# rampasek/GraphGPS

Measured on NVIDIA H100. Metric: graphs/sec GPSLayer fwd+bwd, higher is better.
Workload: dtype f32

## Files before the change

graphgps_b200/_lib.py:

```python
from __future__ import annotations

import ctypes as C
import os

import torch

_HERE = os.path.dirname(os.path.abspath(__file__))
LIB_PATH = os.path.join(_HERE, "libgps_b200.so")

GPS_OK, GPS_ERR_ARG, GPS_ERR_UNSUPPORTED, GPS_ERR_CUDA = 0, -1, -2, -3
LOCAL = {"None": 0, "CustomGatedGCN": 1, "GINE": 2, "GCN": 3, "GAT": 4, "GENConv": 5, "PNA": 6}
GLOBAL = {"None": 0, "Transformer": 1, "Performer": 2, "BigBird": 3}
GLOBAL_BIGBIRD = GLOBAL["BigBird"]
BIGBIRD_ACT = {"relu": 0, "sigmoid": 1}
ACT = {"relu": 0, "gelu": 1}
PRECISION = {"fp32": 0, "bf16": 1}
NORM = {"batch": 0, "none": 1}
FLAG_GRADS_ZEROED, FLAG_GRADS_ACCUMULATE = 1, 2

_fp = C.c_void_p


class GpsGraph(C.Structure):
    _fields_ = [("N", C.c_int64), ("E", C.c_int64), ("B", C.c_int64),
# ... 247 lines not shown
    "gps_pna_aggregate_forward": (C.c_int, [C.POINTER(GpsGraph), _i64, _fp, _fp, _i64, _fp, _fp, _fp, _fp]),
    "gps_pna_aggregate_backward": (C.c_int, [C.POINTER(GpsGraph), _i64, _fp, _fp, _fp, _fp, _fp, _i64, _fp, _fp]),
    "gps_performer_prep": (C.c_int, [C.POINTER(GpsGraph), _i64, _i64, _i64, _fp, _fp, _fp, _fp, _fp, _fp]),
    "gps_performer_features_forward": (C.c_int, [C.POINTER(GpsGraph), _i64, _i64, _i64, _fp, _fp, _fp, _fp, _fp, _fp,
                                                 _fp, _fp]),
    "gps_performer_attention_forward": (C.c_int, [C.POINTER(GpsGraph), _i64, _i64, _i64, _i32, _fp, _fp, _fp, _fp, _fp,
                                                  _fp, _fp, _fp]),
    "gps_performer_attention_backward": (C.c_int, [C.POINTER(GpsGraph), _i64, _i64, _i64, _i32, _fp, _fp, _fp, _fp,
                                                   _fp, _fp, _fp, _fp, _fp, _fp, _fp, _fp, _fp, _fp, _fp]),
    "gps_performer_features_backward": (C.c_int, [C.POINTER(GpsGraph), _i64, _i64, _i64, _i32, _fp, _fp, _fp, _fp, _fp,
                                                  _fp, _fp, _fp, _fp, _fp, _fp, _fp, _fp]),
    "gps_attention_forward": (C.c_int, [C.POINTER(GpsGraph), _i64, _i64, _fp, _fp, _fp, _i64, _fp, _i64, _fp,
                                        _f32, _u64, _u64, _fp]),
    "gps_attention_backward": (C.c_int, [C.POINTER(GpsGraph), _i64, _i64, _fp, _fp, _fp, _i64, _fp, _fp, _i64,
                                         _fp, _fp, _fp, _fp, _fp, _i64, _f32, _u64, _u64, _fp]),
    "gps_attention_forward_tc": (C.c_int, [C.POINTER(GpsGraph), _i64, _i64, _fp, _fp, _i64, _fp, _i64, _fp, _f32, _u64, _u64,
                                           _i32, _fp]),
    "gps_attention_forward_biased": (C.c_int, [C.POINTER(GpsGraph), _i64, _i64, _fp, _fp, _fp, _i64, _fp, _i64, _fp,
                                               _f32, _u64, _u64, C.POINTER(GpsAttnBias), _fp]),
    "gps_attention_forward_tc_biased": (C.c_int, [C.POINTER(GpsGraph), _i64, _i64, _fp, _fp, _i64, _fp, _i64, _fp, _f32,
                                                  _u64, _u64, _i32, C.POINTER(GpsAttnBias), _fp]),
    "gps_attention_backward_biased": (C.c_int, [C.POINTER(GpsGraph), _i64, _i64, _fp, _fp, _fp, _i64, _fp, _fp, _i64,
                                                _fp, _fp, _fp, _fp, _fp, _i64, _f32, _u64, _u64, C.POINTER(GpsAttnBias),
                                                _fp]),
    "gps_dropout_mask": (C.c_int, [_fp, _i64, _i64, _f32, _u64, _u64, _i32, _fp]),
    "gps_to_planes": (C.c_int, [_fp, _i64, _i64, _i64, _fp, _fp, _i64, _fp]),
    "gps_gemm_planes": (C.c_int, [_fp, _fp, _i64, _i32, _fp, _fp, _i64, _i32, _fp, _i64, _fp, _fp, _i64, _i64, _i64, _i64,
                                  _i32, _i32, _fp, _fp]),
    "gps_gemm_epilogue": (C.c_int, [C.POINTER(GpsGemmArgs), _i32, _fp]),
    "gps_fallback_count": (C.c_ulonglong, []),
    "gps_launch_count": (C.c_ulonglong, []),
    "gps_debug_set": (None, [C.c_int]),
    "gps_debug_tma": (None, [C.c_int, _fp]),
    "gps_debug_attn": (None, [_fp]),
}

_lib = None


def load():
    global _lib
    if _lib is not None:
        return _lib
    if not os.path.exists(LIB_PATH):
        raise RuntimeError(
            f"{LIB_PATH} not found: build it with `python -m graphgps_b200.build` "
            "(nvcc, sm_90a). graphgps_b200 has no CPU/eager fallback.")
    lib = C.CDLL(LIB_PATH)
    for name, (res, args) in SYMBOLS.items():
        fn = getattr(lib, name)
        fn.restype = res
        fn.argtypes = args
    if lib.gps_abi_version() != 4:
        raise RuntimeError("libgps_b200.so ABI version mismatch")
    _lib = lib
    return lib


class GpsError(RuntimeError):
    pass


def check(rc: int, what: str):
    if rc == GPS_OK:
        return
    msg = load().gps_last_error().decode("utf-8", "replace")
# ... 10 lines not shown
```

graphgps_b200/csrc/gemm.cuh:

```cuda
#pragma once
#include <cuda.h>

#include "common.cuh"

namespace gps {

struct GemmParams {
  int M = 0, N = 0, K = 0;
  const float* A = nullptr; int lda = 0; int ta = 0;
  const float* B = nullptr; int ldb = 0; int tb = 0;
  float* C = nullptr; int ldc = 0;
  const float* bias = nullptr;
  float* C_pre = nullptr; int ldpre = 0;
  int act = -1;
  const float* mask_src = nullptr; int ldmask = 0; int mask_act = -1;
  int mask_is_post = 0;
  float p_drop = 0.f; uint64_t seed = 0, offset = 0; int site = 0;
  const unsigned long long* offset_dev = nullptr;
  float p_drop2 = 0.f; int site2 = 0;
  const float* R1 = nullptr; int ldr1 = 0;
  const float* R2 = nullptr; int ldr2 = 0;
  double* stats = nullptr;
  int splitk = 1;
  float* colsum_a = nullptr;
  int precision = GPS_PREC_FP32;
  Planes Ap, Bp, Cp;
  int cp_hd = 0, cp_hd_pad = 0;
};

struct ToPlanesItem { const float* src; int64_t ld; int rows; int cols; Planes dst; };
int to_planes(const ToPlanesItem* items, int n, cudaStream_t stream);
int gemm_tma(const GemmParams& p, cudaStream_t stream);
int make_tensor_map(const __nv_bfloat16* hi, const __nv_bfloat16* lo, int planes, int64_t rows, int64_t cols, int64_t ld,
                    int box_rows, CUtensorMap* out);
void gemm_tma_set_force_bn(int bn);
void gemm_tma_set_trace(unsigned long long* buf);

int gemm_simt(const GemmParams& p, cudaStream_t stream);
int gemm_tc(const GemmParams& p, cudaStream_t stream);
void gemm_tc_set_debug(int v);
int gemm(const GemmParams& p, cudaStream_t stream);

}
```

graphgps_b200/csrc/gemm_tma.cu:

```cuda
#include <cooperative_groups.h>
#include <cuda.h>
#include <cuda_bf16.h>

#include <mutex>
#include <unordered_map>

#include "gemm.cuh"
#include "tc_ptx.cuh"

namespace gps {

namespace {

using namespace tc;
namespace cgrp = cooperative_groups;

constexpr int BM = 128;
constexpr int BK = 64;
constexpr int kEpiWarps = 8;
constexpr int kTmaWarp = 8;
constexpr int kThreads = 288;
constexpr int kATile = BM * BK * 2;
constexpr int kBlock = 64 * BK * 2;
constexpr int kMaxSplits = 8;

struct TmaArgs {
  GemmParams p;
  int BN, nb_blocks, stages, kb_per_split, planes;
  unsigned long long* trace;
};

__device__ __forceinline__ unsigned long long gtimer() {
  unsigned long long t;
  asm volatile("mov.u64 %0, %globaltimer;" : "=l"(t));
  return t;
}
#define GPS_TRACE(slot)                                                                         \
  do {                                                                                          \
    if (a.trace && cta_lin < 256) a.trace[cta_lin * 16 + (slot)] = gtimer();                    \
  } while (0)

template <bool A_MN, bool B_MN, int BN_T, bool SPLIT>
__global__ void __launch_bounds__(kThreads, BN_T == 64 ? 2 : 1)
k_gemm_tma(const __grid_constant__ CUtensorMap tmA, const __grid_constant__ CUtensorMap tmB, const TmaArgs a) {
  extern __shared__ __align__(1024) uint8_t smem_raw[];
  const GemmParams& p = a.p;
  uint8_t* smem = reinterpret_cast<uint8_t*>((reinterpret_cast<uintptr_t>(smem_raw) + 1023) & ~(uintptr_t)1023);
  const int planes = a.planes;
  const int b_tile = B_MN ? a.nb_blocks * kBlock : BN_T * 128;
  const int stage_bytes = planes * (kATile + b_tile);
  const int S = a.stages;
  uint64_t* bars = reinterpret_cast<uint64_t*>(smem + (size_t)S * stage_bytes);
  float* red = reinterpret_cast<float*>(bars + 2 * S + 2);
  float* ctot = red + 16 * 16 * 8;
  const int nsplit = (int)gridDim.z;

  const int tid = threadIdx.x, warp = tid >> 5, lane = tid & 31;
  const int m0 = blockIdx.y * BM, n0 = blockIdx.x * a.BN;
  const int nkb_total = (p.K + BK - 1) / BK;
  const int kb_begin = blockIdx.z * a.kb_per_split;
  const int kb_end = min(nkb_total, kb_begin + a.kb_per_split);
  const int nkb = kb_end - kb_begin;
  const bool do_colsum = A_MN && p.colsum_a != nullptr && blockIdx.x == 0;
  const int cta_lin = (blockIdx.z * gridDim.y + blockIdx.y) * gridDim.x + blockIdx.x;

  if (tid == 0) {
    GPS_TRACE(0);
    if (a.trace && cta_lin < 256) {
      unsigned smid;
// ... 108 lines not shown
      __syncwarp();
      if (i > 0 && lane == 0) mbar_arrive(smem_u32(&bars[S + (i - 1) % S]));
    }
    wgmma_wait<0>();
    reg_fence<BN_T / 2>(acc);
    if (tid == 0) GPS_TRACE(4);
    if (do_colsum) {
#pragma unroll
      for (int e = 0; e < 8; ++e) red[(kq * 16 + cm) * 8 + e] = csum[e];
    }
    asm volatile("bar.sync 1, 256;" ::: "memory");
    if (do_colsum && tid < 128) {
      const int cmr = tid >> 3, e = tid & 7;
      float tot = 0.f;
#pragma unroll
      for (int o = 0; o < 16; ++o) tot += red[(o * 16 + cmr) * 8 + e];
      const int gm = m0 + cmr * 8 + e;
      if (nsplit > 1) ctot[cmr * 8 + e] = tot;
      else if (gm < p.M) atomicAdd(&p.colsum_a[gm], tot);
    }
    if (tid == 0) GPS_TRACE(5);
    float* stage = reinterpret_cast<float*>(smem);
    const int sld = a.BN + 4;
    {
      const int r = wg * 64 + (warp & 3) * 16 + (lane >> 2);
      const int c = 2 * (lane & 3);
#pragma unroll
      for (int j = 0; j < BN_T / 8; ++j) {
        *reinterpret_cast<float2*>(stage + r * sld + 8 * j + c) = make_float2(acc[4 * j], acc[4 * j + 1]);
        *reinterpret_cast<float2*>(stage + (r + 8) * sld + 8 * j + c) = make_float2(acc[4 * j + 2], acc[4 * j + 3]);
      }
    }
    asm volatile("bar.sync 1, 256;" ::: "memory");
    const int RB = (BM + nsplit - 1) / nsplit;
    const int lo = (int)blockIdx.z * RB, hi = min(BM, lo + RB);
    if (nsplit > 1) {
      cgrp::cluster_group cluster = cgrp::this_cluster();
      cluster.sync();
      const int c4n = a.BN >> 2;
      for (int idx = tid; idx < (hi - lo) * c4n; idx += kEpiWarps * 32) {
        const int r = lo + idx / c4n, c = (idx % c4n) * 4;
        float4 sum = f4zero();
        for (int k = 0; k < nsplit; ++k)
          sum = f4add(sum, *reinterpret_cast<const float4*>(cluster.map_shared_rank(stage, k) + r * sld + c));
        *reinterpret_cast<float4*>(stage + r * sld + c) = sum;
      }
      if (do_colsum && blockIdx.z == 0 && tid < 128 && m0 + tid < p.M) {
        float tot = 0.f;
        for (int k = 0; k < nsplit; ++k) tot += cluster.map_shared_rank(ctot, k)[tid];
        atomicAdd(&p.colsum_a[m0 + tid], tot);
      }
      cluster.sync();
    }
    const int G = a.BN >> 2;
    const int rpp = kEpiWarps * 32 / G;
    const int rip = tid / G, cg = tid - rip * G;
    const int col = n0 + cg * 4;
    const bool col_ok = rip < rpp && col < p.N;
    const int rows_here = min(BM, p.M - m0);
    const bool colstats = p.stats != nullptr;
    if (col_ok) {
      const int nrows = rip < rows_here ? (rows_here - rip + rpp - 1) / rpp : 0;
      const int64_t row0 = m0 + rip;
      float* sp = stage + rip * sld + cg * 4;
      const int s_st = rpp * sld;
      float* cp = p.C ? p.C + row0 * p.ldc + col : nullptr;
      const int64_t c_st = (int64_t)rpp * p.ldc;
      const float* r1 = p.R1 ? p.R1 + row0 * p.ldr1 + col : nullptr;
      const int64_t r1_st = (int64_t)rpp * p.ldr1;
      const float* r2 = p.R2 ? p.R2 + row0 * p.ldr2 + col : nullptr;
      const int64_t r2_st = (int64_t)rpp * p.ldr2;
      if (p.splitk > 1) {
        for (int r = lo + rip; r < min(hi, rows_here); r += rpp) {
          const int64_t row = m0 + r;
          float4 w = *reinterpret_cast<const float4*>(stage + r * sld + cg * 4);
          if (p.R1) w = f4add(w, ld4(p.R1 + row * p.ldr1 + col));
          if (p.R2) w = f4add(w, ld4(p.R2 + row * p.ldr2 + col));
          atomicAdd(reinterpret_cast<float4*>(p.C + row * p.ldc + col), w);
        }
      } else {
        const bool fast = !p.C_pre && !(p.mask_src && !p.mask_is_post) && p.p_drop == 0.f && p.p_drop2 == 0.f &&
                          (p.act < 0 || p.act == GPS_ACT_RELU);
        const float4 bb = p.bias ? ld4(p.bias + col) : f4zero();
        const float* mk = p.mask_src ? p.mask_src + row0 * p.ldmask + col : nullptr;
        const int64_t mk_st = (int64_t)rpp * p.ldmask;
        int pcol = col, npad = 0;
        if (p.cp_hd > 0) {
          const int hq = col / p.cp_hd, cw = col - hq * p.cp_hd;
          pcol = hq * p.cp_hd_pad + cw;
          npad = (cw + 4 == p.cp_hd) ? p.cp_hd_pad - p.cp_hd : 0;
        }
        __nv_bfloat16* ph = p.Cp.hi ? p.Cp.hi + row0 * p.Cp.ld + pcol : nullptr;
        __nv_bfloat16* pl = p.Cp.lo ? p.Cp.lo + row0 * p.Cp.ld + pcol : nullptr;
        const int64_t p_st = (int64_t)rpp * p.Cp.ld;
        const bool relu = p.act == GPS_ACT_RELU;
        if (fast) {
          for (int k = 0; k < nrows; k += 4) {
// ... 45 lines not shown
              }
            }
          }
        } else {
          const uint64_t drop_off = p.offset + ((p.p_drop > 0.f || p.p_drop2 > 0.f) && p.offset_dev ? *p.offset_dev : 0ull);
          for (int k = 0; k < nrows; ++k) {
            const int64_t row = row0 + (int64_t)k * rpp;
            float4 w = f4add(*reinterpret_cast<const float4*>(sp + k * s_st), bb);
            if (p.C_pre) st4(p.C_pre + row * p.ldpre + col, w);
            if (p.act >= 0) w = make_float4(act_fwd_rt(p.act, w.x), act_fwd_rt(p.act, w.y), act_fwd_rt(p.act, w.z), act_fwd_rt(p.act, w.w));
            if (mk) {
              const float4 ms = ld4(mk + k * mk_st);
              if (p.mask_is_post) {
                w.x = ms.x > 0.f ? w.x : 0.f; w.y = ms.y > 0.f ? w.y : 0.f; w.z = ms.z > 0.f ? w.z : 0.f; w.w = ms.w > 0.f ? w.w : 0.f;
              } else {
                w.x *= act_bwd_rt(p.mask_act, ms.x); w.y *= act_bwd_rt(p.mask_act, ms.y);
                w.z *= act_bwd_rt(p.mask_act, ms.z); w.w *= act_bwd_rt(p.mask_act, ms.w);
              }
            }
            if (p.p_drop2 > 0.f) w = f4mul(w, dropout_scale4(p.p_drop2, p.seed, drop_off, p.site2, ((uint64_t)row * (uint64_t)p.N + col) >> 2));
            if (p.p_drop > 0.f) w = f4mul(w, dropout_scale4(p.p_drop, p.seed, drop_off, p.site, ((uint64_t)row * (uint64_t)p.N + col) >> 2));
            if (r1) w = f4add(w, ld4(r1 + k * r1_st));
            if (r2) w = f4add(w, ld4(r2 + k * r2_st));
            if (cp) st4(cp + k * c_st, w);
            if (ph) {
              planes_store4(p.Cp, row, pcol, w);
              for (int z = 0; z < npad; z += 4) planes_store4(p.Cp, row, pcol + 4 + z, f4zero());
            }
            if (colstats) *reinterpret_cast<float4*>(sp + k * s_st) = w;
          }
        }
      }
    }
    if (colstats) {
      asm volatile("bar.sync 1, 256;" ::: "memory");
      for (int t = tid; t < 16 * G; t += kEpiWarps * 32) {
        const int y = t / G, g = t - y * G, c = n0 + g * 4;
        if (c >= p.N) continue;
        float4 s1 = f4zero(), s2 = f4zero();
        for (int r = y; r < rows_here; r += 16) {
          const float4 w = *reinterpret_cast<const float4*>(stage + r * sld + g * 4);
          s1 = f4add(s1, w);
          s2 = f4fma(w, w, s2);
        }
        float* o = stage + y * sld + g * 4;
        *reinterpret_cast<float4*>(o) = s1;
        *reinterpret_cast<float4*>(o + 16 * sld) = s2;
      }
      asm volatile("bar.sync 1, 256;" ::: "memory");
      if (tid < G && n0 + tid * 4 < p.N) {
        float4 t[2] = {f4zero(), f4zero()};
        for (int y = 0; y < 16; ++y) {
          t[0] = f4add(t[0], *reinterpret_cast<const float4*>(stage + y * sld + tid * 4));
          t[1] = f4add(t[1], *reinterpret_cast<const float4*>(stage + (y + 16) * sld + tid * 4));
        }
        const int c0 = n0 + tid * 4;
        auto add4 = [&](double* dst, float4 v) {
          atomic_add_f64(dst + 0, (double)v.x); atomic_add_f64(dst + 1, (double)v.y);
          atomic_add_f64(dst + 2, (double)v.z); atomic_add_f64(dst + 3, (double)v.w);
        };
        add4(p.stats + c0, t[0]);
        add4(p.stats + (int64_t)p.N + c0, t[1]);
      }
    }
  }

  if (tid == 0) GPS_TRACE(6);
  if (a.trace) {
    __syncthreads();
    if (tid == 0) GPS_TRACE(7);
  }
}

// ... 81 lines not shown
  static bool attr_done = false;
  if (!attr_done) {
    GPS_CUDA(cudaFuncSetAttribute(k_gemm_tma<A_MN, B_MN, BN_T, SPLIT>, cudaFuncAttributeMaxDynamicSharedMemorySize,
                                  227 * 1024));
    attr_done = true;
  }
  if (grid.z == 1) {
    k_gemm_tma<A_MN, B_MN, BN_T, SPLIT><<<grid, kThreads, smem, stream>>>(tA, tB, a);
  } else {
    cudaLaunchConfig_t cfg = {};
    cfg.gridDim = grid;
    cfg.blockDim = dim3(kThreads);
    cfg.dynamicSmemBytes = smem;
    cfg.stream = stream;
    cudaLaunchAttribute attr[1];
    attr[0].id = cudaLaunchAttributeClusterDimension;
    attr[0].val.clusterDim.x = 1;
    attr[0].val.clusterDim.y = 1;
    attr[0].val.clusterDim.z = grid.z;
    cfg.attrs = attr;
    cfg.numAttrs = 1;
    GPS_CUDA(cudaLaunchKernelEx(&cfg, k_gemm_tma<A_MN, B_MN, BN_T, SPLIT>, tA, tB, a));
  }
  GPS_LAUNCH_CHECK();
  return GPS_OK;
}
template <bool A_MN, bool B_MN, int BN_T>
int launch(const CUtensorMap& tA, const CUtensorMap& tB, const TmaArgs& a, dim3 grid, size_t smem, cudaStream_t stream) {
  return a.planes == 2 ? launch1<A_MN, B_MN, BN_T, true>(tA, tB, a, grid, smem, stream)
                       : launch1<A_MN, B_MN, BN_T, false>(tA, tB, a, grid, smem, stream);
}

int g_tma_force_bn = 0;
unsigned long long* g_tma_trace = nullptr;

}

void gemm_tma_set_force_bn(int bn) { g_tma_force_bn = bn; }
void gemm_tma_set_trace(unsigned long long* buf) { g_tma_trace = buf; }

int gemm_tma(const GemmParams& p, cudaStream_t stream) {
  if (p.M <= 0 || p.N <= 0) return GPS_OK;
  if (p.K <= 0 || !p.Ap.hi || !p.Bp.hi) return GPS_ERR_UNSUPPORTED;
  const bool split = p.precision == GPS_PREC_FP32;
  const int planes = split ? 2 : 1;
  if (split && (!p.Ap.lo || !p.Bp.lo)) return GPS_ERR_UNSUPPORTED;
  if (!aligned16(p.Ap.hi) || !aligned16(p.Bp.hi) || p.Ap.ld % 8 || p.Bp.ld % 8 || p.N % 4) return GPS_ERR_UNSUPPORTED;
  if (split && (!aligned16(p.Ap.lo) || !aligned16(p.Bp.lo))) return GPS_ERR_UNSUPPORTED;
  if ((p.C && (!aligned16(p.C) || p.ldc % 4)) || (!p.C && !p.Cp.hi)) return GPS_ERR_UNSUPPORTED;
  if (p.Cp.hi && (p.Cp.ld % 4 || (reinterpret_cast<uintptr_t>(p.Cp.hi) & 7) || (p.Cp.lo && (reinterpret_cast<uintptr_t>(p.Cp.lo) & 7))))
    return GPS_ERR_UNSUPPORTED;
  if ((p.bias && !aligned16(p.bias)) || (p.R1 && (!aligned16(p.R1) || p.ldr1 % 4)) ||
      (p.R2 && (!aligned16(p.R2) || p.ldr2 % 4)) || (p.mask_src && (!aligned16(p.mask_src) || p.ldmask % 4)) ||
      (p.C_pre && (!aligned16(p.C_pre) || p.ldpre % 4)))
    return GPS_ERR_UNSUPPORTED;
  if (p.splitk > 1 && (p.bias || p.act >= 0 || p.mask_src || p.stats || p.C_pre || p.p_drop != 0.f || p.p_drop2 != 0.f ||
                       p.Cp.hi || !p.C)) {
    set_error("gemm: split-K supports the plain fp32 product (+ residuals) only");
    return GPS_ERR_ARG;
  }
  if (p.colsum_a && !p.ta) {
    set_error("gemm: colsum_a needs ta == 1");
    return GPS_ERR_ARG;
  }
  const int mt = (int)ceil_div(p.M, BM);
  const int nkb = (int)ceil_div(p.K, BK);
  const int splits_hint = p.splitk > 1 ? min(kMaxSplits, min(p.splitk, nkb)) : 1;
  const auto width_ok = [&](int bn) {
    return bn == 64 || bn == 128 || (bn == 152 && !p.tb) || (bn == 256 && !p.ta);
  };
  int bestBN = 0;
  long bestCost = 0;
  for (const int bn : {64, 128, 152, 256}) {
    if (!width_ok(bn)) continue;
    const long tiles = (long)mt * ceil_div(p.N, bn) * splits_hint;
    const long cost = bn != 64 ? ceil_div(tiles, (long)kNumSMs) * bn : tiles <= kNumSMs ? 64 : ceil_div(tiles, 2L * kNumSMs) * 160;
    if (!bestBN || cost <= bestCost) { bestCost = cost; bestBN = bn; }
  }
  if (g_tma_force_bn) {
    if (!width_ok(g_tma_force_bn)) return GPS_ERR_UNSUPPORTED;
    bestBN = g_tma_force_bn;
  }
  TmaArgs a;
  a.p = p;
  a.BN = bestBN;
  a.nb_blocks = a.BN / 64;
  a.planes = planes;
  const bool narrow = a.nb_blocks == 1;
  const int stage_bytes = planes * (kATile + (p.tb ? a.nb_blocks * kBlock : a.BN * 128));
  const int fixed = 1024  + 1024  + 16 * 16 * 8 * 4 + 128 * 4;
  int stages = ((narrow ? 112 : 226) * 1024 - fixed) / stage_bytes;
  if (stages > 8) stages = 8;
  if (stages < 2) return GPS_ERR_UNSUPPORTED;
  GPS_REQUIRE((size_t)stages * stage_bytes >= (size_t)BM * (a.BN + 4) * 4, GPS_ERR_ARG,
              "gemm_tma: BN %d: the staging tile does not fit the operand stages", a.BN);
  a.stages = stages;
  int splitk = p.splitk > 1 ? p.splitk : 1;
  if (splitk > kMaxSplits) splitk = kMaxSplits;
  if (splitk > nkb) splitk = nkb;
  a.kb_per_split = (int)ceil_div(nkb, splitk);
  splitk = (int)ceil_div(nkb, a.kb_per_split);
  a.p.splitk = p.splitk > 1 ? 2 : 1;
  a.trace = g_tma_trace;
  const bool amn = p.ta != 0, bmn = p.tb != 0;
  CUtensorMap tA, tB;
  GPS_TRY(tensor_map(p.Ap.hi, p.Ap.lo, planes, amn ? p.K : p.M, amn ? p.M : p.K, p.Ap.ld, amn ? 64 : BM, &tA));
  GPS_TRY(tensor_map(p.Bp.hi, p.Bp.lo, planes, bmn ? p.K : p.N, bmn ? p.N : p.K, p.Bp.ld, bmn ? 64 : a.BN, &tB));
  const size_t smem = (size_t)stages * stage_bytes + fixed;
  dim3 grid((unsigned)ceil_div(p.N, a.BN), (unsigned)mt, (unsigned)splitk);
#define GPS_TMA_CASE(AM, BMN)                                                                              \
  if (amn == AM && bmn == BMN) {                                                                           \
    if (a.BN == 64) return launch<AM, BMN, 64>(tA, tB, a, grid, smem, stream);                            \
    if (a.BN == 128) return launch<AM, BMN, 128>(tA, tB, a, grid, smem, stream);                          \
  }
  GPS_TMA_CASE(false, false)
  GPS_TMA_CASE(false, true)
  GPS_TMA_CASE(true, false)
  GPS_TMA_CASE(true, true)
#undef GPS_TMA_CASE
  if (a.BN == 152 && !bmn)
    return amn ? launch<true, false, 152>(tA, tB, a, grid, smem, stream) : launch<false, false, 152>(tA, tB, a, grid, smem, stream);
  if (a.BN == 256 && !amn)
    return bmn ? launch<false, true, 256>(tA, tB, a, grid, smem, stream) : launch<false, false, 256>(tA, tB, a, grid, smem, stream);
  return GPS_ERR_UNSUPPORTED;
}

namespace {
struct ToPlanesDesc {
  ToPlanesItem it[16];
  int start[17];
  int n;
};
__global__ void k_to_planes(ToPlanesDesc d) {
  int item = 0;
  while (item + 1 < d.n && (int)blockIdx.x >= d.start[item + 1]) ++item;
  const ToPlanesItem& it = d.it[item];
  const int cpr = (it.cols + 7) >> 3;
  const int64_t total = (int64_t)it.rows * cpr;
  const int64_t idx = ((int64_t)blockIdx.x - d.start[item]) * blockDim.x + threadIdx.x;
  if (idx >= total) return;
  const int64_t r = idx / cpr;
  const int c = (int)(idx - r * cpr) * 8;
// ... 43 lines not shown
```

graphgps_b200/csrc/layer.cu:

```cuda
#include <stdarg.h>
#include <string.h>

#include <algorithm>
#include <atomic>

#include "layer_ops.cuh"

namespace gps {

int perf_supported(int64_t dim_head, int64_t features);
int64_t perf_mp();
int perf_index_range(int64_t N, int64_t H);
int perf_prep(const float* P, int64_t m, float* Pn, const GpsGraph& g, int64_t H, int* nmax, float* gmax, int* argk,
              cudaStream_t st);
int perf_features_fwd(float* fq, float* fk, const float* Q, const float* K, const GpsGraph& g, int64_t H, int64_t m,
                      float* gmax, int* argq, int* argk, cudaStream_t st);
int perf_linattn_fwd(const GpsGraph& g, int64_t H, int64_t m, const int* nmax, const float* qf, const float* kf,
                     const float* V, const float* gmax, float* O, cudaStream_t st);
int perf_linattn_bwd(const GpsGraph& g, int64_t H, int64_t m, const int* nmax, const float* qf, const float* kf,
                     const float* V, const float* gmax, const float* gO, float* g_qf, float* g_kf, float* gV,
                     float* ggmax, cudaStream_t st);
int perf_features_bwd(float* g_fq, float* g_fk, const float* fq, const float* fk, const float* Q, const float* K,
                      float* gQ, float* gK, const GpsGraph& g, int64_t H, int64_t m, const int* argq, const int* argk,
                      const float* ggmax, float* gmrow, bool pairwise, cudaStream_t st);
// ... 978 lines not shown
  const GpsPna& pna = a->pna;
  GPS_TRY(make_plan(a, &P, true));
  GPS_REQUIRE(a->saved && a->workspace, GPS_ERR_ARG, "saved/workspace buffers are required");
  GPS_REQUIRE(a->workspace_bytes >= P.bwd_bytes, GPS_ERR_ARG, "workspace too small (%lld < %lld)",
              (long long)a->workspace_bytes, (long long)P.bwd_bytes);
  GPS_TRY(check_params(a, P));
  GPS_REQUIRE(a->grad_x_out && a->grad_x, GPS_ERR_ARG, "grad_x_out / grad_x are required");
  GPS_REQUIRE(!P.gat || P.E == 0 || a->grad_edge_attr, GPS_ERR_ARG, "grad_edge_attr is required for GAT");
  GPS_REQUIRE(!P.gen || P.E == 0 || a->grad_edge_attr, GPS_ERR_ARG, "grad_edge_attr is required for GENConv");
  GPS_REQUIRE(!P.pna || P.E == 0 || a->grad_edge_attr, GPS_ERR_ARG, "grad_edge_attr is required for PNA");
  const int64_t N = P.N, E = P.E, d = P.d;
  const int act = a->act;
  DropCfg nodrop;
  auto sums = [&](int which) { return P.bsums + (int64_t)which * 2 * d; };
  GPS_CUDA(cudaMemsetAsync(P.bsums, 0, (size_t)P.nbn * 2 * d * sizeof(double), st));
  if (P.gen) GPS_CUDA(cudaMemsetAsync(P.gen_bsums, 0, (size_t)2 * 2 * d * sizeof(double), st));
  Side* sd;
  GPS_TRY(side_stream(&sd));
  cudaStream_t s2 = sd->s;
  auto wfork = [&](cudaStream_t from) -> int { return sd->order(from, s2); };
  const bool two_branches = P.loc && P.glob;
  cudaStream_t sa = two_branches ? sd->s3 : st;
  cudaStream_t se = sd->s4;
  auto record_ev = [&](void* ev, cudaStream_t s) -> int {
    if (!ev) return GPS_OK;
    cudaStreamCaptureStatus cs = cudaStreamCaptureStatusNone;
    GPS_CUDA(cudaStreamIsCapturing(s, &cs));
    GPS_CUDA(cudaEventRecordWithFlags((cudaEvent_t)ev, s, cs == cudaStreamCaptureStatusActive ? cudaEventRecordExternal
                                                                                               : cudaEventRecordDefault));
    return GPS_OK;
  };
  auto early_done = [&]() -> int { return record_ev(a->ev_grads_early, s2); };
  auto mid_done = [&]() -> int { return record_ev(a->ev_grads_mid, s2); };
  const bool gx_splitk = P.Wy >= 1024 && N > 0;
  if (P.Wy) {
    GPS_TRY(wfork(st));
    GPS_CUDA(cudaMemsetAsync(P.gWcat, 0, (size_t)(P.Wy * d + P.Wy) * sizeof(float), s2));
  }
  if (gx_splitk) GPS_CUDA(cudaMemsetAsync(a->grad_x, 0, (size_t)(N * d) * sizeof(float), st));

  if (P.gated) {
    GPS_TRY(sd->order(st, se));
    BnView ve = bn_view(P, BN_E, a->bn_edge_e);
    if (a->grad_edge_out && E > 0) {
      GPS_TRY(bn_bwd_reduce(a->grad_edge_out, d, P.ehat, d, E, d, ve, act, P.drop(GPS_SITE_GCN_E), sums(BN_E), se));
      GPS_TRY(bn_bwd_apply(a->grad_edge_out, d, P.ehat, d, E, d, ve, act, P.drop(GPS_SITE_GCN_E), sums(BN_E), P.g_e, d,
                           a->bn_edge_e.grad_weight, a->bn_edge_e.grad_bias, se, P.grads_accumulate));
    } else {
      if (E > 0) GPS_CUDA(cudaMemsetAsync(P.g_e, 0, (size_t)(E * d) * sizeof(float), se));
      if (a->bn_edge_e.grad_weight && !P.grads_prezeroed)
        GPS_CUDA(cudaMemsetAsync(a->bn_edge_e.grad_weight, 0, d * sizeof(float), se));
      if (a->bn_edge_e.grad_bias && !P.grads_prezeroed)
        GPS_CUDA(cudaMemsetAsync(a->bn_edge_e.grad_bias, 0, d * sizeof(float), se));
    }
  }

  const float* g_t = P.nonorm ? a->grad_x_out : P.g_t;
  if (!P.nonorm) {
    BnView v2 = bn_view(P, BN_2, a->norm2);
    GPS_TRY(bn_bwd_reduce(a->grad_x_out, d, P.t, d, N, d, v2, -1, nodrop, sums(BN_2), st));
    GPS_TRY(bn_bwd_apply(a->grad_x_out, d, P.t, d, N, d, v2, -1, nodrop, sums(BN_2), P.g_t, d, a->norm2.grad_weight,
                         a->norm2.grad_bias, st, P.grads_accumulate, P.gt_p));
  } else if (!(P.dropout.p > 0.f) && P.gt_p.hi && N > 0) {
    ToPlanesItem it{g_t, d, (int)N, (int)d, P.gt_p};
    GPS_TRY(to_planes(&it, 1, st));
  }
  const float* g_xloc = P.nonorm ? P.g_s : P.g_xloc;
  const Planes g_xloc_p = P.nonorm ? P.gs_p : P.gl1_p;
  const float* g_hA = P.nonorm ? P.g_s : P.g_hA;
  const Planes g_hA_p = P.nonorm ? P.gs_p : P.ghA_p;

  {
// ... 228 lines not shown
    GPS_TRY(wfork(st));
    GPS_TRY(linear_wgrad(P, g_l, {P.pna_h, d, P.pna_h_p}, N, d, d, pna.lin.grad_weight, pna.lin.grad_bias, s2));
    GPS_TRY(linear_wgrad(P, g_h, {P.pna_Z, 4 * d, P.pna_Z_p}, N, d, 4 * d, pna.post.grad_weight, pna.post.grad_bias,
                         s2));
    GPS_TRY(gemm(linear_dgrad(P, N, 4 * d, d, g_h, {pna.post.weight, 4 * d, P.post_p}, P.pna_gZ, 4 * d), st));
    GPS_TRY(pna_bwd(a->graph, d, P.pna_gZ, P.pna_arg, g_xloc, P.pna_gq, P.pna_gq_p, P.gY1, P.Wy, P.gY1_p, P.g_xl, st));
    const Operand g_q{P.pna_gq, d, P.pna_gq_p};
    float* g_F = P.pna_gF;
    float* g_c = P.pna_gF + d * P.de;
    GPS_TRY(wfork(st));
    GPS_CUDA(cudaMemsetAsync(g_F, 0, (size_t)(d * P.de + d) * sizeof(float), s2));
    GPS_TRY(wgrad_add(P, g_q, {a->edge_attr, P.de, P.e_p}, E, d, P.de, g_F, g_c, s2));
    GPS_TRY(pna_fold_bwd(pna.pre.weight, pna.edge_encoder.weight, pna.edge_encoder.bias, g_F, g_c, d, P.de,
                         pna.pre.grad_weight, pna.pre.grad_bias, pna.edge_encoder.grad_weight,
                         pna.edge_encoder.grad_bias, P.grads_accumulate, s2));
    GPS_TRY(mid_done());
    if (E > 0)
      GPS_TRY(gemm(linear_dgrad(P, E, P.de, d, g_q, {P.pna_F, P.de, P.pna_F_p}, a->grad_edge_attr, P.de), st));
    g_x_local = P.g_xl;
  }

  if (two_branches) GPS_TRY(sd->order(sa, st));

  if (P.Wy) {
    const Operand gY1{P.gY1, P.Wy, P.gY1_p};
    GPS_TRY(wfork(st));
    GPS_TRY(wgrad_add(P, gY1, {a->x, d, P.x_p}, N, P.Wy, d, P.gWcat, P.gbcat, s2));
    PackDesc pdsc = pack_desc(P);
    k_unpack<<<(unsigned)P.Wy, 128, 0, s2>>>(pdsc, P.gWcat, P.gbcat, P.grads_accumulate ? 1 : 0);
    GPS_LAUNCH_CHECK();
    GemmParams g = linear_dgrad(P, N, d, P.Wy, gY1, {P.Wcat, d, P.Wcat_p}, a->grad_x, d);
    g.R1 = g_x_local; g.ldr1 = (int)d;
    g.R2 = P.attn ? g_hA : (P.perf ? P.g_xp : (P.bb ? P.bb_gx : nullptr)); g.ldr2 = (int)d;
    if (gx_splitk) g.splitk = 4;
    GPS_TRY(gemm(g, st));
  } else if (g_x_local) {
    GPS_TRY(add3(g_x_local, d, P.perf ? P.g_xp : nullptr, d, nullptr, 0, a->grad_x, d, N, d, st));
  } else {
    GPS_TRY(add3(P.g_xp, d, nullptr, 0, nullptr, 0, a->grad_x, d, N, d, st));
  }
  GPS_TRY(sd->join(st));
  if (P.gated) GPS_TRY(sd->order(se, st));
  GPS_TRY(record_ev(a->ev_grads_done, st));
  return GPS_OK;
}

}

using namespace gps;

extern "C" const char* gps_last_error(void) { return g_err; }
extern "C" int gps_abi_version(void) { return GPS_ABI_VERSION; }
extern "C" const char* gps_build_arch(void) { return "sm_90a"; }
extern "C" unsigned long long gps_launch_count(void) { return g_launches.load(); }
extern "C" unsigned long long gps_fallback_count(void) { return g_fallbacks.load(); }

extern "C" int gps_to_planes(const float* src, int64_t ld, int64_t rows, int64_t cols, void* hi, void* lo, int64_t ldp,
                             void* stream) {
  GPS_REQUIRE(src && hi, GPS_ERR_ARG, "gps_to_planes: null argument");
  ToPlanesItem it{src, ld, (int)rows, (int)cols, Planes{(__nv_bfloat16*)hi, (__nv_bfloat16*)lo, ldp}};
  return to_planes(&it, 1, (cudaStream_t)stream);
}

extern "C" int gps_gemm_planes(const void* A_hi, const void* A_lo, int64_t lda, int32_t ta, const void* B_hi,
                               const void* B_lo, int64_t ldb, int32_t tb, float* C, int64_t ldc, void* C_hi, void* C_lo,
                               int64_t ldcp, int64_t M, int64_t N, int64_t K, int32_t splitk, int32_t precision,
                               float* colsum_a, void* stream) {
// ... 22 lines not shown
  GemmParams g;
  g.M = (int)a->M; g.N = (int)a->N; g.K = (int)a->K;
  g.A = a->A; g.lda = (int)a->lda; g.ta = a->ta;
  g.B = a->B; g.ldb = (int)a->ldb; g.tb = a->tb;
  g.Ap = Planes{(__nv_bfloat16*)a->Ap.hi, (__nv_bfloat16*)a->Ap.lo, a->Ap.ld};
  g.Bp = Planes{(__nv_bfloat16*)a->Bp.hi, (__nv_bfloat16*)a->Bp.lo, a->Bp.ld};
  g.Cp = Planes{(__nv_bfloat16*)a->Cp.hi, (__nv_bfloat16*)a->Cp.lo, a->Cp.ld};
  g.C = a->C; g.ldc = (int)a->ldc; g.cp_hd = a->cp_hd; g.cp_hd_pad = a->cp_hd_pad;
  g.bias = a->bias; g.C_pre = a->C_pre; g.ldpre = (int)a->ldpre; g.act = a->act;
  g.mask_src = a->mask_src; g.ldmask = (int)a->ldmask; g.mask_act = a->mask_act; g.mask_is_post = a->mask_is_post;
  g.p_drop = a->p_drop; g.site = a->site; g.p_drop2 = a->p_drop2; g.site2 = a->site2;
  g.seed = a->seed; g.offset = a->offset; g.offset_dev = a->offset_dev;
  g.R1 = a->R1; g.ldr1 = (int)a->ldr1; g.R2 = a->R2; g.ldr2 = (int)a->ldr2;
  g.stats = a->stats; g.colsum_a = a->colsum_a; g.splitk = a->splitk < 1 ? 1 : a->splitk; g.precision = a->precision;
  const cudaStream_t st = (cudaStream_t)stream;
  int rc;
  switch (impl) {
    case 1: rc = gemm_simt(g, st); break;
    case 2: rc = gemm_tc(g, st); break;
    case 3: rc = gemm_tma(g, st); break;
    default: return gemm(g, st);
  }
  if (rc == GPS_ERR_UNSUPPORTED)
    set_error("gps_gemm_epilogue: impl %d does not take M=%d N=%d K=%d (ta=%d tb=%d) with these alignments", impl, g.M,
              g.N, g.K, g.ta, g.tb);
  return rc;
}

extern "C" void gps_debug_set(int v) { gemm_tc_set_debug(v); }
extern "C" void gps_debug_tma(int force_bn, void* trace) {
  gemm_tma_set_force_bn(force_bn);
  gemm_tma_set_trace((unsigned long long*)trace);
}
extern "C" void gps_debug_attn(void* buf) { attention_tc_set_debug((float*)buf); }

extern "C" int gps_layer_plan(const GpsLayerArgs* args, GpsLayerPlan* plan) {
  GPS_REQUIRE(args && plan, GPS_ERR_ARG, "gps_layer_plan: null argument");
  Plan P;
  GPS_TRY(make_plan(args, &P, false));
  plan->saved_bytes = P.saved_bytes;
  plan->fwd_workspace_bytes = P.fwd_bytes;
  plan->bwd_workspace_bytes = P.bwd_bytes;
  plan->wplanes_bytes = P.wplanes_bytes;
  return GPS_OK;
}

extern "C" int gps_layer_forward(const GpsLayerArgs* args, void* stream) {
  GPS_REQUIRE(args, GPS_ERR_ARG, "gps_layer_forward: null args");
  return layer_forward(args, (cudaStream_t)stream);
}

extern "C" int gps_layer_backward(const GpsLayerArgs* args, void* stream) {
  GPS_REQUIRE(args, GPS_ERR_ARG, "gps_layer_backward: null args");
  return layer_backward(args, (cudaStream_t)stream);
}

static int bb_stage(const GpsGraph* g, int64_t heads, int64_t hd, const GpsBigBird* bb, const char* what) {
  GPS_REQUIRE(g && bb, GPS_ERR_ARG, "%s: null argument", what);
  GPS_REQUIRE(hd >= 1 && heads >= 1, GPS_ERR_ARG, "%s: heads and hd must be >= 1", what);
  return bb_check(heads * hd, heads, bb);
}

extern "C" int gps_bigbird_attention_forward(const GpsGraph* g, int64_t heads, int64_t hd, const GpsBigBird* bb,
                                             const float* Q, const float* K, const float* V, int64_t ld, float* O,
                                             int64_t ldo, float* lse, void* stream) {
  GPS_TRY(bb_stage(g, heads, hd, bb, "bigbird_attention_forward"));
// ... 411 lines not shown
```

include/gps_b200.h:

```cpp
#ifndef GPS_B200_H_
#define GPS_B200_H_

#include <stdint.h>

#ifdef __cplusplus
extern "C" {
#endif

#define GPS_ABI_VERSION 4

enum { GPS_OK = 0, GPS_ERR_ARG = -1, GPS_ERR_UNSUPPORTED = -2, GPS_ERR_CUDA = -3 };

enum { GPS_LOCAL_NONE = 0, GPS_LOCAL_GATEDGCN = 1, GPS_LOCAL_GINE = 2, GPS_LOCAL_GCN = 3, GPS_LOCAL_GAT = 4,
       GPS_LOCAL_GENCONV = 5, GPS_LOCAL_PNA = 6 };
enum { GPS_GLOBAL_NONE = 0, GPS_GLOBAL_TRANSFORMER = 1, GPS_GLOBAL_PERFORMER = 2,
       GPS_GLOBAL_BIGBIRD = 3 };
enum { GPS_ACT_RELU = 0, GPS_ACT_GELU = 1 };
enum { GPS_PREC_FP32 = 0, GPS_PREC_BF16 = 1 };
enum { GPS_NORM_BATCH = 0, GPS_NORM_NONE = 1 };

const char* gps_last_error(void);
int gps_abi_version(void);
const char* gps_build_arch(void);
unsigned long long gps_launch_count(void);
void gps_debug_set(int v);
void gps_debug_tma(int force_bn, void* trace);
void gps_debug_attn(void* buf);

typedef struct {
  int64_t N, E, B;
  const int32_t* dst_ptr;
  const int32_t* dst_src;
  const int32_t* dst_eid;
  const int32_t* src_ptr;
  const int32_t* src_dst;
  const int32_t* src_eid;
  const int32_t* graph_ptr;
} GpsGraph;

int64_t gps_graph_bytes(int64_t N, int64_t E, int64_t B);
int gps_graph_build(const int64_t* edge_index, const int64_t* batch, int64_t N, int64_t E,
                    int64_t B, void* storage, int64_t storage_bytes, GpsGraph* out,
                    void* stream);

typedef struct {
  const float* weight;
  const float* bias;
  float* running_mean;
  float* running_var;
  int64_t* num_batches_tracked;
  float* grad_weight;
  float* grad_bias;
} GpsBatchNorm;

typedef struct {
  const float* weight;
  const float* bias;
  float* grad_weight;
  float* grad_bias;
// ... 497 lines not shown
```

Measured before the change: 357,500.

## Auto-select TMA GEMM split-K count and split the epilogue rows across the cluster

The TMA GEMM now chooses its split-K factor with a cost model over wave counts and per-split k-blocks, so small-M/N GEMMs can spread K across more CTAs automatically. The explicit split-K path for the grad_x dgrad, along with its memset, is removed in favour of this automatic choice. After the DSMEM reduction, each cluster rank now writes back and computes column stats only for its own row slice instead of every rank covering the whole tile. The cluster reduction also gets an unrolled multi-load variant for wider tiles. The risk is that the cost-model heuristic picks split counts that add cluster sync and reduction overhead on GEMMs that were fine unsplit.

```diff
diff --git a/graphgps_b200/_lib.py b/graphgps_b200/_lib.py
--- a/graphgps_b200/_lib.py
+++ b/graphgps_b200/_lib.py
@@ -303,6 +303,7 @@
     "gps_launch_count": (C.c_ulonglong, []),
     "gps_debug_set": (None, [C.c_int]),
     "gps_debug_tma": (None, [C.c_int, _fp]),
+    "gps_debug_tma_splits": (None, [C.c_int]),
     "gps_debug_attn": (None, [_fp]),
 }
 
diff --git a/graphgps_b200/csrc/gemm.cuh b/graphgps_b200/csrc/gemm.cuh
--- a/graphgps_b200/csrc/gemm.cuh
+++ b/graphgps_b200/csrc/gemm.cuh
@@ -34,6 +34,7 @@
 int make_tensor_map(const __nv_bfloat16* hi, const __nv_bfloat16* lo, int planes, int64_t rows, int64_t cols, int64_t ld,
                     int box_rows, CUtensorMap* out);
 void gemm_tma_set_force_bn(int bn);
+void gemm_tma_set_force_splits(int s);
 void gemm_tma_set_trace(unsigned long long* buf);
 
 int gemm_simt(const GemmParams& p, cudaStream_t stream);
diff --git a/graphgps_b200/csrc/gemm_tma.cu b/graphgps_b200/csrc/gemm_tma.cu
--- a/graphgps_b200/csrc/gemm_tma.cu
+++ b/graphgps_b200/csrc/gemm_tma.cu
@@ -35,6 +35,15 @@
   asm volatile("mov.u64 %0, %globaltimer;" : "=l"(t));
   return t;
 }
+__device__ __forceinline__ int2 split_rows() {
+  int z, nz;
+  asm volatile("mov.u32 %0, %%ctaid.z;" : "=r"(z));
+  asm volatile("mov.u32 %0, %%nctaid.z;" : "=r"(nz));
+  const int RB = ((BM + nz - 1) / nz + 15) & ~15;
+  const int lo = min(BM, z * RB);
+  return make_int2(lo, min(BM, lo + RB));
+}
+
 #define GPS_TRACE(slot)                                                                         \
   do {                                                                                          \
     if (a.trace && cta_lin < 256) a.trace[cta_lin * 16 + (slot)] = gtimer();                    \
@@ -209,18 +218,43 @@
       }
     }
     asm volatile("bar.sync 1, 256;" ::: "memory");
-    const int RB = (BM + nsplit - 1) / nsplit;
-    const int lo = (int)blockIdx.z * RB, hi = min(BM, lo + RB);
+    const int lo = split_rows().x, hi = split_rows().y;
     if (nsplit > 1) {
       cgrp::cluster_group cluster = cgrp::this_cluster();
       cluster.sync();
       const int c4n = a.BN >> 2;
-      for (int idx = tid; idx < (hi - lo) * c4n; idx += kEpiWarps * 32) {
-        const int r = lo + idx / c4n, c = (idx % c4n) * 4;
-        float4 sum = f4zero();
-        for (int k = 0; k < nsplit; ++k)
-          sum = f4add(sum, *reinterpret_cast<const float4*>(cluster.map_shared_rank(stage, k) + r * sld + c));
-        *reinterpret_cast<float4*>(stage + r * sld + c) = sum;
+      const int n4 = max(0, min(hi, p.M - m0) - lo) * c4n;
+      constexpr int U = BN_T == 64 ? 1 : 4, kStep = kEpiWarps * 32;
+      if constexpr (U == 1) {
+        for (int idx = tid; idx < n4; idx += kStep) {
+          const int o = (lo + idx / c4n) * sld + (idx % c4n) * 4;
+          float4 sum = f4zero();
+          for (int k = 0; k < nsplit; ++k)
+            sum = f4add(sum, *reinterpret_cast<const float4*>(cluster.map_shared_rank(stage, k) + o));
+          *reinterpret_cast<float4*>(stage + o) = sum;
+        }
+      } else {
+        for (int b = tid; b < n4; b += U * kStep) {
+          int off[U];
+          float4 sum[U];
+#pragma unroll
+          for (int u = 0; u < U; ++u) {
+            const int idx = min(b + u * kStep, n4 - 1);
+            off[u] = (lo + idx / c4n) * sld + (idx % c4n) * 4;
+            sum[u] = f4zero();
+          }
+          for (int k = 0; k < nsplit; ++k) {
+            const float* src = cluster.map_shared_rank(stage, k);
+            float4 v[U];
+#pragma unroll
+            for (int u = 0; u < U; ++u) v[u] = *reinterpret_cast<const float4*>(src + off[u]);
+#pragma unroll
+            for (int u = 0; u < U; ++u) sum[u] = f4add(sum[u], v[u]);
+          }
+#pragma unroll
+          for (int u = 0; u < U; ++u)
+            if (b + u * kStep < n4) *reinterpret_cast<float4*>(stage + off[u]) = sum[u];
+        }
       }
       if (do_colsum && blockIdx.z == 0 && tid < 128 && m0 + tid < p.M) {
         float tot = 0.f;
@@ -235,11 +269,12 @@
     const int col = n0 + cg * 4;
     const bool col_ok = rip < rpp && col < p.N;
     const int rows_here = min(BM, p.M - m0);
+    const int row_end = min(hi, rows_here);
     const bool colstats = p.stats != nullptr;
     if (col_ok) {
-      const int nrows = rip < rows_here ? (rows_here - rip + rpp - 1) / rpp : 0;
-      const int64_t row0 = m0 + rip;
-      float* sp = stage + rip * sld + cg * 4;
+      const int nrows = lo + rip < row_end ? (row_end - lo - rip + rpp - 1) / rpp : 0;
+      const int64_t row0 = m0 + lo + rip;
+      float* sp = stage + (lo + rip) * sld + cg * 4;
       const int s_st = rpp * sld;
       float* cp = p.C ? p.C + row0 * p.ldc + col : nullptr;
       const int64_t c_st = (int64_t)rpp * p.ldc;
@@ -351,13 +386,15 @@
         }
       }
     }
-    if (colstats) {
+    const int2 own = split_rows();
+    const int slo = own.x, send = min(own.y, min(BM, p.M - m0));
+    if (colstats && slo < send) {
       asm volatile("bar.sync 1, 256;" ::: "memory");
       for (int t = tid; t < 16 * G; t += kEpiWarps * 32) {
         const int y = t / G, g = t - y * G, c = n0 + g * 4;
         if (c >= p.N) continue;
         float4 s1 = f4zero(), s2 = f4zero();
-        for (int r = y; r < rows_here; r += 16) {
+        for (int r = slo + y; r < send; r += 16) {
           const float4 w = *reinterpret_cast<const float4*>(stage + r * sld + g * 4);
           s1 = f4add(s1, w);
           s2 = f4fma(w, w, s2);
@@ -505,11 +542,13 @@
 }
 
 int g_tma_force_bn = 0;
+int g_tma_force_splits = 0;
 unsigned long long* g_tma_trace = nullptr;
 
 }
 
 void gemm_tma_set_force_bn(int bn) { g_tma_force_bn = bn; }
+void gemm_tma_set_force_splits(int s) { g_tma_force_splits = s; }
 void gemm_tma_set_trace(unsigned long long* buf) { g_tma_trace = buf; }
 
 int gemm_tma(const GemmParams& p, cudaStream_t stream) {
@@ -538,18 +577,47 @@
   }
   const int mt = (int)ceil_div(p.M, BM);
   const int nkb = (int)ceil_div(p.K, BK);
-  const int splits_hint = p.splitk > 1 ? min(kMaxSplits, min(p.splitk, nkb)) : 1;
+  const auto splits_of = [&](int s) {
+    s = max(1, min(kMaxSplits, min(s, nkb)));
+    return (int)ceil_div(nkb, ceil_div(nkb, s));
+  };
   const auto width_ok = [&](int bn) {
     return bn == 64 || bn == 128 || (bn == 152 && !p.tb) || (bn == 256 && !p.ta);
   };
-  int bestBN = 0;
-  long bestCost = 0;
-  for (const int bn : {64, 128, 152, 256}) {
-    if (!width_ok(bn)) continue;
-    const long tiles = (long)mt * ceil_div(p.N, bn) * splits_hint;
-    const long cost = bn != 64 ? ceil_div(tiles, (long)kNumSMs) * bn : tiles <= kNumSMs ? 64 : ceil_div(tiles, 2L * kNumSMs) * 160;
-    if (!bestBN || cost <= bestCost) { bestCost = cost; bestBN = bn; }
-  }
+  const auto wave_cost = [&](int bn, long ctas) -> long {
+    return bn != 64 ? ceil_div(ctas, (long)kNumSMs) * bn : ctas <= kNumSMs ? 64 : ceil_div(ctas, 2L * kNumSMs) * 160;
+  };
+  const auto best_width = [&](int s, long* cost_out) {
+    int best = 0;
+    long best_cost = 0;
+    for (const int bn : {64, 128, 152, 256}) {
+      if (!width_ok(bn)) continue;
+      const long cost = wave_cost(bn, (long)mt * ceil_div(p.N, bn) * s);
+      if (!best || cost <= best_cost) { best_cost = cost; best = bn; }
+    }
+    if (cost_out) *cost_out = best_cost;
+    return best;
+  };
+  int nsplit = 1;
+  if (p.splitk > 1) {
+    nsplit = splits_of(p.splitk);
+  } else if (g_tma_force_splits > 0) {
+    nsplit = splits_of(g_tma_force_splits);
+  } else {
+    long best_cost = 0;
+    for (int s = 1; s <= kMaxSplits; ++s) {
+      if (splits_of(s) != s) continue;
+      const int kbps = (int)ceil_div(nkb, s);
+      if (s > 1 && nkb - (s - 1) * kbps < 2) continue;
+      long wc = 0;
+      const int bn = best_width(s, &wc);
+      if (s > 1 && (long)mt * ceil_div(p.N, bn) * s > kNumSMs) continue;
+      if (bn == 64) wc = max(wc, 128L);
+      const long cost = wc * (4L * kbps + 28 + (s > 1 ? 20 : 0));
+      if (s == 1 || cost < best_cost) { best_cost = cost; nsplit = s; }
+    }
+  }
+  int bestBN = best_width(p.splitk > 1 ? min(kMaxSplits, min(p.splitk, nkb)) : nsplit, nullptr);
   if (g_tma_force_bn) {
     if (!width_ok(g_tma_force_bn)) return GPS_ERR_UNSUPPORTED;
     bestBN = g_tma_force_bn;
@@ -568,11 +636,7 @@
   GPS_REQUIRE((size_t)stages * stage_bytes >= (size_t)BM * (a.BN + 4) * 4, GPS_ERR_ARG,
               "gemm_tma: BN %d: the staging tile does not fit the operand stages", a.BN);
   a.stages = stages;
-  int splitk = p.splitk > 1 ? p.splitk : 1;
-  if (splitk > kMaxSplits) splitk = kMaxSplits;
-  if (splitk > nkb) splitk = nkb;
-  a.kb_per_split = (int)ceil_div(nkb, splitk);
-  splitk = (int)ceil_div(nkb, a.kb_per_split);
+  a.kb_per_split = (int)ceil_div(nkb, nsplit);
   a.p.splitk = p.splitk > 1 ? 2 : 1;
   a.trace = g_tma_trace;
   const bool amn = p.ta != 0, bmn = p.tb != 0;
@@ -580,7 +644,7 @@
   GPS_TRY(tensor_map(p.Ap.hi, p.Ap.lo, planes, amn ? p.K : p.M, amn ? p.M : p.K, p.Ap.ld, amn ? 64 : BM, &tA));
   GPS_TRY(tensor_map(p.Bp.hi, p.Bp.lo, planes, bmn ? p.K : p.N, bmn ? p.N : p.K, p.Bp.ld, bmn ? 64 : a.BN, &tB));
   const size_t smem = (size_t)stages * stage_bytes + fixed;
-  dim3 grid((unsigned)ceil_div(p.N, a.BN), (unsigned)mt, (unsigned)splitk);
+  dim3 grid((unsigned)ceil_div(p.N, a.BN), (unsigned)mt, (unsigned)nsplit);
 #define GPS_TMA_CASE(AM, BMN)                                                                              \
   if (amn == AM && bmn == BMN) {                                                                           \
     if (a.BN == 64) return launch<AM, BMN, 64>(tA, tB, a, grid, smem, stream);                            \
diff --git a/graphgps_b200/csrc/layer.cu b/graphgps_b200/csrc/layer.cu
--- a/graphgps_b200/csrc/layer.cu
+++ b/graphgps_b200/csrc/layer.cu
@@ -1034,12 +1034,10 @@
   };
   auto early_done = [&]() -> int { return record_ev(a->ev_grads_early, s2); };
   auto mid_done = [&]() -> int { return record_ev(a->ev_grads_mid, s2); };
-  const bool gx_splitk = P.Wy >= 1024 && N > 0;
   if (P.Wy) {
     GPS_TRY(wfork(st));
     GPS_CUDA(cudaMemsetAsync(P.gWcat, 0, (size_t)(P.Wy * d + P.Wy) * sizeof(float), s2));
   }
-  if (gx_splitk) GPS_CUDA(cudaMemsetAsync(a->grad_x, 0, (size_t)(N * d) * sizeof(float), st));
 
   if (P.gated) {
     GPS_TRY(sd->order(st, se));
@@ -1334,7 +1332,6 @@
     GemmParams g = linear_dgrad(P, N, d, P.Wy, gY1, {P.Wcat, d, P.Wcat_p}, a->grad_x, d);
     g.R1 = g_x_local; g.ldr1 = (int)d;
     g.R2 = P.attn ? g_hA : (P.perf ? P.g_xp : (P.bb ? P.bb_gx : nullptr)); g.ldr2 = (int)d;
-    if (gx_splitk) g.splitk = 4;
     GPS_TRY(gemm(g, st));
   } else if (g_x_local) {
     GPS_TRY(add3(g_x_local, d, P.perf ? P.g_xp : nullptr, d, nullptr, 0, a->grad_x, d, N, d, st));
@@ -1423,6 +1420,7 @@
   gemm_tma_set_force_bn(force_bn);
   gemm_tma_set_trace((unsigned long long*)trace);
 }
+extern "C" void gps_debug_tma_splits(int splits) { gemm_tma_set_force_splits(splits); }
 extern "C" void gps_debug_attn(void* buf) { attention_tc_set_debug((float*)buf); }
 
 extern "C" int gps_layer_plan(const GpsLayerArgs* args, GpsLayerPlan* plan) {
diff --git a/include/gps_b200.h b/include/gps_b200.h
--- a/include/gps_b200.h
+++ b/include/gps_b200.h
@@ -25,6 +25,7 @@
 unsigned long long gps_launch_count(void);
 void gps_debug_set(int v);
 void gps_debug_tma(int force_bn, void* trace);
+void gps_debug_tma_splits(int splits);
 void gps_debug_attn(void* buf);
 
 typedef struct {
```

Result: faster. 368,500, median of 6 (+3.1%).
